# Weepingchestnut/SAVSR

Hardware: AMD Instinct MI355X
Metric: HR Mpixels/sec (Vid4-shape x4, 7-frame window) (higher is better)
Workload: dtype f32 (bf16x3 split products, fp32 accumulate)

## Files before the change

### savsr_amd/csrc/conv_common.hpp

```cpp
#pragma once
#include "common.hpp"

namespace savsr {

struct ConvParams {
    const float* src[SAVSR_MAX_SRC];
    int src_pix[SAVSR_MAX_SRC];
    const unsigned short* wimg;
    const float* bias;
    int act;
    float slope;
    const float* mul_px;
    const float* res1;
    int res1_pix;
    const float* res2;
    int res2_pix;
    float res2_scale;
    float* out;
    int out_pix;
    float* pool;
    int pool_stride;
};

#ifndef SAVSR_CONV_MAX_BATCH
#define SAVSR_CONV_MAX_BATCH 24
#endif
constexpr int CONV_MAX_BATCH = SAVSR_CONV_MAX_BATCH;
constexpr int CONV_WIDE_MIN_TILES = 200;
constexpr int CONV_WIDE_MIN_TILES_TP = 100;
#ifndef SAVSR_CONV_BLOCKS
#define SAVSR_CONV_BLOCKS 256
#endif
constexpr int CONV_PERSISTENT_BLOCKS = SAVSR_CONV_BLOCKS;
#ifndef WY_STRIP
#define WY_STRIP 1
#endif
struct MultiConvParams {
    ConvParams c[CONV_MAX_BATCH];
    int h, w, cout, nchunk, src_ch;
    int nconv, ncob, ntx, nty;
    int wy_tiles, wy_full, wy_strip_l2;
};
static_assert(sizeof(MultiConvParams) <= 4096, "MultiConvParams is passed by value as the conv kernels' argument: at most 4 KB");

int launch_conv_wy(const MultiConvParams& mp, hipStream_t st, bool f16);
int conv_wy_prepare_device();

typedef _Float16 f16x8 __attribute__((ext_vector_type(8)));
typedef _Float16 f16x4 __attribute__((ext_vector_type(4)));

#define SAVSR_GLOBAL __attribute__((address_space(1)))
__device__ __forceinline__ f32x4 ldg4(const float* base, unsigned byte_off) {
    return *(const SAVSR_GLOBAL f32x4*)((const SAVSR_GLOBAL char*)base + byte_off);
}
__device__ __forceinline__ float ldg1(const float* base, unsigned idx) {
    return *((const SAVSR_GLOBAL float*)base + idx);
}
#ifndef CONV_ST
#define CONV_ST 1
#endif
__device__ __forceinline__ void stg4(float* base, unsigned byte_off, const f32x4& v) {
#if CONV_ST == 1
    __builtin_nontemporal_store(v, (SAVSR_GLOBAL f32x4*)((SAVSR_GLOBAL char*)base + byte_off));
#else
    *(SAVSR_GLOBAL f32x4*)((SAVSR_GLOBAL char*)base + byte_off) = v;
#endif
}
__device__ __forceinline__ float vmax_raw(float a, float b) {
    float r;
    asm("v_max_f32 %0, %1, %2" : "=v"(r) : "v"(a), "v"(b));
    return r;
}
__device__ __forceinline__ void stg1(float* base, unsigned idx, float v) {
    *((SAVSR_GLOBAL float*)base + idx) = v;
}

}
```

### savsr_amd/csrc/conv_mfma.hip

```cpp
#include "conv_common.hpp"

#include <type_traits>


#ifndef CONV_BUF
#define CONV_BUF 1
#endif

namespace savsr {

[[maybe_unused]] constexpr int STAMP_BLOCKS = 1024, STAMP_N = 6;
#if defined(SAVSR_DIAG)
#define CONV_HAS_STAMPS 1
__device__ long long g_conv_stamps[STAMP_BLOCKS * STAMP_N];
__device__ int g_conv_stamps_on = 0;
#else
#define CONV_HAS_STAMPS 0
#endif
__device__ __attribute__((aligned(16))) const float g_conv_zero16[4] = {0.f, 0.f, 0.f, 0.f};

__device__ __forceinline__ void stamp(int on, int slot) {
#if CONV_HAS_STAMPS
    if (on == 1 && threadIdx.x == 0 && blockIdx.x < STAMP_BLOCKS)
        g_conv_stamps[blockIdx.x * STAMP_N + slot] = (slot == 5) ? (long long)__builtin_amdgcn_s_memrealtime() : (long long)__builtin_amdgcn_s_memtime();
#endif
}

template <int KS, int NT, int PXT, bool DIAG, bool F16>
__global__ __launch_bounds__(512) void conv_bf16x3_kernel(const MultiConvParams mp) {
    constexpr int TH = CONV_TH * PXT, NTHR = 64 * CONV_TH;
    constexpr int TAPS = KS * KS, HALO = KS / 2;
    constexpr int KC = conv_kc(KS), KSTEPS = KC / 16;
    constexpr int IR = TH + 2 * HALO, IC = CONV_TW + 2 * HALO, NPX = IR * IC;
    constexpr int B_PART = KSTEPS * 2 * NPX;
    constexpr int B_UNITS = 2 * B_PART;
    constexpr int W_UNITS = TAPS * KSTEPS * NT * 2 * 64;
    constexpr int W_IMG = F16 ? W_UNITS / 2 : W_UNITS;
    constexpr int PER = KSTEPS * 4;
    constexpr int B_ITEMS = NPX * PER;
    constexpr int B_IT = (B_ITEMS + NTHR - 1) / NTHR;
    constexpr int W_IT = (W_UNITS + NTHR - 1) / NTHR;
    constexpr int STEPS = TAPS * KSTEPS;
    constexpr int COT = 32 * NT;
    constexpr int EPS = 36;

    extern __shared__ __attribute__((aligned(16))) unsigned char smem_raw[];
    bf16x8* smem = reinterpret_cast<bf16x8*>(smem_raw);
    constexpr bool EP_ALIAS = PXT > 1;
    static_assert(!EP_ALIAS || B_UNITS * 16 >= CONV_TH * 32 * EPS * 4, "aliased epilogue slices must fit one input buffer");

    const int tid = threadIdx.x, lane = tid & 63, wave = tid >> 6, half = lane >> 5, px = lane & 31;
    [[maybe_unused]] const int prio_group = __builtin_amdgcn_readfirstlane(wave >> 2);
    const int tiles_per_cob = mp.ntx * mp.nty;
    const int total = mp.nconv * mp.ncob * tiles_per_cob;
#if CONV_HAS_STAMPS
    const int dbg_all = DIAG ? __builtin_amdgcn_readfirstlane(g_conv_stamps_on) : 0;
#else
    static_assert(!DIAG, "DIAG kernels exist in the instrumented library only");
    const int dbg_all = 0;
#endif
    const int stamps_on = dbg_all & 15;
    const bool dbg_nostage = dbg_all & 16, dbg_nofrag = dbg_all & 32;
    const bool dbg_nost = dbg_all & 64, dbg_nolds = dbg_all & 128;

    f32x4 b_reg[B_IT];
    [[maybe_unused]] const unsigned tid16 = (unsigned)tid * 16u;

    struct TileInfo { int conv, cob, x0, y0, tx, ty; };
    auto decode = [&](int tile) {
        const int cc = tile / tiles_per_cob, rem = tile - cc * tiles_per_cob;
        const int ty = rem / mp.ntx, tx = rem - ty * mp.ntx;
        TileInfo ti;
        ti.conv = cc / mp.ncob;
        ti.cob = cc - ti.conv * mp.ncob;
        ti.x0 = tx * CONV_TW;
        ti.y0 = ty * TH;
        ti.tx = tx;
        ti.ty = ty;
        return ti;
    };
    const int H = mp.h, W = mp.w;
    const float* st_base = nullptr;
    const f32x4* st_w = nullptr;
    int st_pix = 0, st_cb = 0, st_src = 0, st_conv = 0;
#if CONV_BUF
    constexpr unsigned OOB = 0x80000000u;
    unsigned st_voff[B_IT];
    int st_x0 = 0, st_y0 = 0;
    auto stage_offsets = [&]() {
#pragma unroll
        for (int i = 0; i < B_IT; ++i) {
            const int e = tid + i * NTHR;
            const int pl = e / PER, c8 = e - pl * PER;
            const int r = pl / IC, c = pl - r * IC;
            const int gy = st_y0 - HALO + r, gx = st_x0 - HALO + c;
            const bool ok = (e < B_ITEMS) & ((unsigned)gy < (unsigned)H) & ((unsigned)gx < (unsigned)W);
            const unsigned v = (unsigned)((gy * W + gx) * st_pix + c8 * 4) * 4u;
            st_voff[i] = ok ? v : OOB;
        }
    };
    auto uni = [](int v) { return __builtin_amdgcn_readfirstlane(v); };
    auto uni_ptr = [](const float* q) {
        const unsigned long long a = (unsigned long long)(uintptr_t)q;
        const unsigned lo = (unsigned)__builtin_amdgcn_readfirstlane((int)(unsigned)a), hi = (unsigned)__builtin_amdgcn_readfirstlane((int)(unsigned)(a >> 32));
        return (const float*)(uintptr_t)(((unsigned long long)hi << 32) | lo);
    };
#else
    int st_pixoff[B_IT];
    auto uni = [](int v) { return v; };
    auto uni_ptr = [](const float* q) { return q; };
#endif
    auto stage_begin_tile = [&](const TileInfo& ti) {
        st_conv = ti.conv;
        st_src = 0;
        st_cb = 0;
        st_base = uni_ptr(mp.c[ti.conv].src[0]);
        st_pix = uni(mp.c[ti.conv].src_pix[0]);
        st_w = reinterpret_cast<const f32x4*>(mp.c[ti.conv].wimg) + (long long)ti.cob * mp.nchunk * W_IMG;
#if CONV_BUF
        st_x0 = ti.x0;
        st_y0 = ti.y0;
        stage_offsets();
#else
#pragma unroll
        for (int i = 0; i < B_IT; ++i) {
            const int e = tid + i * NTHR;
            int off = -1;
            if (e < B_ITEMS) {
                const int pl = e / PER;
                const int r = pl / IC, c = pl - r * IC;
                const int gy = ti.y0 - HALO + r, gx = ti.x0 - HALO + c;
                if (gy >= 0 && gy < H && gx >= 0 && gx < W) off = gy * W + gx;
            }
            st_pixoff[i] = off;
        }
#endif
    };
    auto stage_advance = [&]() {
        st_cb += KC;
        st_w += W_IMG;
        if (st_cb >= mp.src_ch) {
            st_cb = 0;
            ++st_src;
            st_base = uni_ptr(mp.c[st_conv].src[st_src]);
#if CONV_BUF
            const int pix_new = uni(mp.c[st_conv].src_pix[st_src]);
            if (pix_new != st_pix) { st_pix = pix_new; stage_offsets(); }
#else
            st_pix = mp.c[st_conv].src_pix[st_src];
#endif
        }
    };
    auto issue_w = [&](int g, int wbuf) {
        const int e = tid + g * NTHR;
// ... 513 lines not shown
    asm volatile("s_waitcnt vmcnt(0)" ::: "memory");
    if (stamps_on == 1) {
        __builtin_amdgcn_s_waitcnt(0);
        stamp(stamps_on, 4);
    }
#if CONV_HAS_STAMPS
    if (stamps_on >= 3 && tid == (stamps_on - 3) * 64 && blockIdx.x < STAMP_BLOCKS)
        for (int i = 0; i < 5; ++i) g_conv_stamps[blockIdx.x * STAMP_N + i] = sec[i];
#endif
}

#ifdef SAVSR_DIAG
static int g_conv_diag_host = 0;
#endif

template <int KS, int NT, int PXT>
constexpr size_t conv_lds_bytes() {
    constexpr int TAPS = KS * KS, HALO = KS / 2, KC = conv_kc(KS), KSTEPS = KC / 16;
    constexpr int NPX = (CONV_TH * PXT + 2 * HALO) * (CONV_TW + 2 * HALO);
    return 16ull * 2 * (2 * KSTEPS * 2 * NPX + TAPS * KSTEPS * NT * 2 * 64) + (PXT > 1 ? 0ull : 4ull * CONV_TH * 32 * 36);
}

template <int KS, int NT, int PXT, bool DIAG, bool F16>
static int launch_conv_impl(const MultiConvParams& mp, hipStream_t st) {
    constexpr size_t lds = conv_lds_bytes<KS, NT, PXT>();
    static_assert(lds <= 160 * 1024, "LDS budget");
    if (int rc = ensure_dynamic_lds(reinterpret_cast<const void*>(&conv_bf16x3_kernel<KS, NT, PXT, DIAG, F16>), (int)lds, "conv")) return rc;
    const int total = mp.nconv * mp.ncob * mp.ntx * mp.nty;
    const int grid = total < CONV_PERSISTENT_BLOCKS ? total : CONV_PERSISTENT_BLOCKS;
    hipLaunchKernelGGL((conv_bf16x3_kernel<KS, NT, PXT, DIAG, F16>), dim3(grid), dim3(64 * CONV_TH), lds, st, mp);
    return check_launch("conv_bf16x3_kernel");
}

template <int KS, int NT, int PXT>
static int launch_conv(const MultiConvParams& mp, hipStream_t st, bool f16) {
    if (f16) return launch_conv_impl<KS, NT, PXT, false, true>(mp, st);
#ifdef SAVSR_DIAG
    if (g_conv_diag_host) return launch_conv_impl<KS, NT, PXT, true, false>(mp, st);
#endif
    return launch_conv_impl<KS, NT, PXT, false, false>(mp, st);
}

template <int KS, int NT, int PXT>
static int conv_attr() {
    if (int rc = ensure_dynamic_lds(reinterpret_cast<const void*>(&conv_bf16x3_kernel<KS, NT, PXT, false, false>), (int)conv_lds_bytes<KS, NT, PXT>(), "conv")) return rc;
    return ensure_dynamic_lds(reinterpret_cast<const void*>(&conv_bf16x3_kernel<KS, NT, PXT, false, true>), (int)conv_lds_bytes<KS, NT, PXT>(), "conv");
}
int conv_prepare_device() {
    if (int rc = conv_attr<3, 2, 2>()) return rc;
    if (int rc = conv_attr<3, 2, 1>()) return rc;
    if (int rc = conv_attr<3, 1, 1>()) return rc;
    if (int rc = conv_attr<1, 2, 1>()) return rc;
    if (int rc = conv_attr<1, 2, 2>()) return rc;
    if (int rc = conv_attr<1, 1, 1>()) return rc;
    return conv_wy_prepare_device();
}

}

using namespace savsr;

#if CONV_HAS_STAMPS
extern "C" int savsr_debug_read_conv_stamps(long long* host, int nblocks) {
    if (!host || nblocks < 1 || nblocks > STAMP_BLOCKS) return fail_arg("debug_read_conv_stamps");
    hipError_t e = hipMemcpyFromSymbol(host, HIP_SYMBOL(g_conv_stamps), sizeof(long long) * STAMP_N * nblocks);
    return e == hipSuccess ? 0 : (int)e;
}
#endif
#ifdef SAVSR_DIAG
extern "C" int savsr_debug_conv_stamps(int enable) {
    g_conv_diag_host = enable;
    hipError_t e = hipMemcpyToSymbol(HIP_SYMBOL(g_conv_stamps_on), &enable, sizeof(int));
    return e == hipSuccess ? 0 : (int)e;
}

#endif

extern "C" int savsr_conv_pool_blocks(int h, int w) {
    return ((w + CONV_TW - 1) / CONV_TW) * ((h + CONV_TH - 1) / CONV_TH);
}

extern "C" int64_t savsr_conv_packed_elems(int cout, int cin, int ksize) {
    if (cout <= 0 || cin <= 0 || (ksize != 1 && ksize != 3)) return -1;
    const int kc = conv_kc(ksize), cot = conv_cot(cout);
    if (cin % kc) return -1;
    const int64_t nchunk = cin / kc, ncob = (cout + cot - 1) / cot;
    return ncob * nchunk * ksize * ksize * kc * cot;
}

extern "C" int64_t savsr_conv_pack_index(int cout, int cin, int ksize, int co, int ci, int tap) {
    const int kc = conv_kc(ksize), cot = conv_cot(cout), nt = cot / 32, ksteps = kc / 16;
    const int64_t nchunk = cin / kc;
    const int cob = co / cot, col = co % cot, t = col / 32, row = col % 32;
    const int chunk = ci / kc, cl = ci % kc, ks = cl / 16, kh = (cl % 16) / 8, j = cl % 8;
    const int64_t group = (((int64_t)(cob * nchunk + chunk) * (ksize * ksize) + tap) * ksteps + ks) * nt + t;
    return group * 512 + (kh * 32 + row) * 8 + j;
}

static int fill_params(const savsr_conv_desc* d, ConvParams& p) {
    if (d->ksize != 1 && d->ksize != 3) return fail_arg("conv: ksize must be 1 or 3");
    const int kc = conv_kc(d->ksize);
    if (d->nsrc < 1 || d->nsrc > SAVSR_MAX_SRC || d->src_ch < kc || d->src_ch % kc) return fail_arg("conv: nsrc / src_ch (multiple of 16, or 32 for 1x1)");
    if (d->cin != d->nsrc * d->src_ch) return fail_arg("conv: cin != nsrc*src_ch");
    if (d->h < 1 || d->w < 1 || d->cout < 1) return fail_arg("conv: shape");
    if (!d->wpacked || !d->out) return fail_arg("conv: null weights/out");
    uintptr_t al = reinterpret_cast<uintptr_t>(d->wpacked);
    uintptr_t al_out = reinterpret_cast<uintptr_t>(d->out) | (uintptr_t)(d->out_pix * 4);
    for (int i = 0; i < SAVSR_MAX_SRC; ++i) {
        const bool on = i < d->nsrc;
        if (on && !d->src[i]) return fail_arg("conv: null source");
        p.src[i] = on ? d->src[i] : nullptr;
        p.src_pix[i] = on ? d->src_pix[i] : 0;
        if (on) al |= reinterpret_cast<uintptr_t>(d->src[i]) | (uintptr_t)(d->src_pix[i] * 4);
    }
    if (d->res1) al_out |= reinterpret_cast<uintptr_t>(d->res1) | (uintptr_t)(d->res1_pix * 4);
    if (d->res2) al_out |= reinterpret_cast<uintptr_t>(d->res2) | (uintptr_t)(d->res2_pix * 4);
    if (d->bias) al |= reinterpret_cast<uintptr_t>(d->bias);
    if ((al & 15) || ((al_out & 15) && d->cout >= 4)) {
        set_error("conv: sources / residuals / bias / out / weights must be 16-byte aligned with pixel strides multiple of 4 floats");
        return SAVSR_E_ALIGN;
    }
    p.wimg = reinterpret_cast<const unsigned short*>(d->wpacked);
    p.bias = d->bias; p.act = d->act; p.slope = d->slope;
    p.mul_px = d->mul_px; p.res1 = d->res1; p.res1_pix = d->res1_pix; p.res2 = d->res2; p.res2_pix = d->res2_pix;
    p.res2_scale = d->res2_scale;
    p.out = d->out; p.out_pix = d->out_pix;
    p.pool = d->pool; p.pool_stride = d->pool_stride;
    if (d->pool && (d->cout % 4 || d->pool_stride < d->cout)) return fail_arg("conv: pool needs cout % 4 == 0 and pool_stride >= cout");
    {
        int64_t max_pix = d->out_pix;
        for (int i = 0; i < d->nsrc; ++i) max_pix = d->src_pix[i] > max_pix ? d->src_pix[i] : max_pix;
        if (d->res1 && d->res1_pix > max_pix) max_pix = d->res1_pix;
        if (d->res2 && d->res2_pix > max_pix) max_pix = d->res2_pix;
        if ((int64_t)d->h * d->w * max_pix * 4 >= (int64_t)1 << 31) return fail_arg("conv: tensors of 2 GiB or more are not supported");
    }
    return 0;
}

static void wy_tile_plan(int h, int per, int algo, MultiConvParams& mp) {
    const int left = h % 16, pairs = (left + 1) / 2;
    mp.wy_strip_l2 = pairs <= 1 ? 0 : (pairs <= 2 ? 1 : 2);
    mp.wy_full = mp.wy_tiles = mp.ntx * mp.nty;
    if (WY_STRIP && left > 0 && left <= 8) {
        const int segs = 8 >> mp.wy_strip_l2;
        const int full = mp.ntx * (mp.nty - 1), tiles = full + (mp.ntx + segs - 1) / segs;
        const int wgs = CONV_PERSISTENT_BLOCKS;
        if (WY_STRIP == 2 || (pairs <= 2 && algo == SAVSR_CONV_WINOGRAD_Y_THROUGHPUT) || (per * tiles + wgs - 1) / wgs < (per * mp.wy_tiles + wgs - 1) / wgs) {
            mp.wy_full = full;
            mp.wy_tiles = tiles;
        }
    }
}

extern "C" int64_t savsr_conv_wy_tile_count(int h, int w, int cout, int nconv, int algo) {
    if (h < 1 || w < 1 || cout < 64 || cout % 64 || nconv < 1 || nconv > CONV_MAX_BATCH ||
        (algo != SAVSR_CONV_WINOGRAD_Y && algo != SAVSR_CONV_WINOGRAD_Y_THROUGHPUT)) return -1;
    MultiConvParams mp;
    mp.ncob = cout / 64;
    mp.ntx = (w + CONV_TW - 1) / CONV_TW;
    mp.nty = (h + 15) / 16;
    wy_tile_plan(h, nconv * mp.ncob, algo, mp);
    return (int64_t)nconv * mp.ncob * mp.wy_tiles;
}

extern "C" int savsr_conv2d_max_batch(void) { return CONV_MAX_BATCH; }

static int conv2d_batch(const savsr_conv_desc* descs, int n, void* stream, bool f16) {
    if (!descs) return fail_arg("conv: null descriptor");
    if (n < 1 || n > CONV_MAX_BATCH) return fail_arg("conv: batch size must be 1..24 (savsr_conv2d_max_batch())");
    MultiConvParams mp;
    for (int i = 0; i < n; ++i) {
        const int rc = fill_params(descs + i, mp.c[i]);
        if (rc) return rc;
        const savsr_conv_desc& a = descs[0];
        const savsr_conv_desc& b = descs[i];
        if (b.ksize != a.ksize || b.nsrc != a.nsrc || b.src_ch != a.src_ch || b.h != a.h || b.w != a.w || b.cout != a.cout || b.algo != a.algo)
            return fail_arg("conv: all convs of a batch must share ksize / nsrc / src_ch / h / w / cout / algo");
    }
    for (int i = n; i < CONV_MAX_BATCH; ++i) mp.c[i] = mp.c[0];
    const savsr_conv_desc* d = descs;
    const int cot = conv_cot(d->cout);
    mp.h = d->h; mp.w = d->w; mp.cout = d->cout;
    mp.nchunk = d->cin / conv_kc(d->ksize);
    mp.src_ch = d->src_ch;
    mp.nconv = n;
    mp.ncob = (d->cout + cot - 1) / cot;
    mp.ntx = (d->w + CONV_TW - 1) / CONV_TW;
    mp.nty = (d->h + CONV_TH - 1) / CONV_TH;
    hipStream_t st = static_cast<hipStream_t>(stream);
    if (d->algo == SAVSR_CONV_WINOGRAD_Y || d->algo == SAVSR_CONV_WINOGRAD_Y_THROUGHPUT) {
        if (d->ksize != 3 || d->cout % 64) return fail_arg("conv: algo WINOGRAD_Y needs ksize 3 and cout a multiple of 64");
        mp.nty = (d->h + 15) / 16;
        wy_tile_plan(d->h, n * mp.ncob, d->algo, mp);
        return launch_conv_wy(mp, st, f16);
    }
    if (d->algo != SAVSR_CONV_DIRECT && d->algo != SAVSR_CONV_DIRECT_THROUGHPUT) return fail_arg("conv: unknown algo");
    const bool wide = cot == 64;
    if (d->ksize == 3 && wide) {
        const int nty2 = (d->h + 2 * CONV_TH - 1) / (2 * CONV_TH);
        if (d->cout % 64 == 0 && n * mp.ncob * mp.ntx * nty2 >= (d->algo == SAVSR_CONV_DIRECT_THROUGHPUT ? CONV_WIDE_MIN_TILES_TP : CONV_WIDE_MIN_TILES)) {
            mp.nty = nty2;
            return launch_conv<3, 2, 2>(mp, st, f16);
        }
        return launch_conv<3, 2, 1>(mp, st, f16);
    }
    if (d->ksize == 3) return launch_conv<3, 1, 1>(mp, st, f16);
    if (wide && d->cout % 64 == 0) {
        const int nty2 = (d->h + 2 * CONV_TH - 1) / (2 * CONV_TH);
        if (n * mp.ncob * mp.ntx * nty2 >= (d->algo == SAVSR_CONV_DIRECT_THROUGHPUT ? CONV_WIDE_MIN_TILES_TP : CONV_WIDE_MIN_TILES)) {
            mp.nty = nty2;
            return launch_conv<1, 2, 2>(mp, st, f16);
        }
    }
    return wide ? launch_conv<1, 2, 1>(mp, st, f16) : launch_conv<1, 1, 1>(mp, st, f16);
}

extern "C" int savsr_conv2d_batch(const savsr_conv_desc* descs, int n, void* stream) { return conv2d_batch(descs, n, stream, false); }
extern "C" int savsr_conv2d_batch_f16(const savsr_conv_desc* descs, int n, void* stream) { return conv2d_batch(descs, n, stream, true); }

extern "C" int savsr_conv2d(const savsr_conv_desc* d, void* stream) { return savsr_conv2d_batch(d, 1, stream); }
```

### savsr_amd/csrc/conv_wy.hip

```cpp
#include "conv_common.hpp"

#include <type_traits>

#ifndef WY_STAMPS
#define WY_STAMPS 0
#endif
#ifndef WY_VALU
#define WY_VALU 6
#endif
#ifndef WY_FAST_EPILOGUE
#define WY_FAST_EPILOGUE 1
#endif
#ifndef WY_BUF
#define WY_BUF 1
#endif

namespace savsr {

namespace wy {
constexpr int TH = 16, TW = 32, NTHR = 512, COT = 64;
[[maybe_unused]] constexpr int IC = TW + 2;
#ifndef WY_ICP
#define WY_ICP 36
#endif
constexpr int ICP = WY_ICP;
constexpr int V_PLANE = 2 * ICP;
constexpr int V_WAVE = 2 * 2 * 2 * V_PLANE;
constexpr int W_HALF = 6 * 2 * 2 * 64;
constexpr int W_PHASE = 2 * W_HALF;
constexpr int EPS = 36;
constexpr int LDS_UNITS = 8 * V_WAVE + 2 * W_HALF;
constexpr size_t LDS_BYTES = 16ull * LDS_UNITS + 4ull * 8 * 32 * EPS;
static_assert(LDS_BYTES <= 160 * 1024, "LDS budget");
}

__device__ __attribute__((aligned(16))) const float g_wy_zero16[4] = {0.f, 0.f, 0.f, 0.f};

#if WY_STAMPS
__device__ long long g_wy_stamps[256 * 8 * 8];
#define WY_KSEC(i) (WY_STAMPS == 2 ? 0 : (i))
#define WY_MARK(i) do { const long long t_now = (long long)__builtin_amdgcn_s_memtime(); wy_sec[i] += t_now - wy_prev; wy_prev = t_now; } while (0)
#if WY_STAMPS == 2
#define WY_EMARK(i) WY_MARK(i)
#endif
#else
#define WY_KSEC(i) (i)
#define WY_MARK(i) do { } while (0)
#endif

typedef float f32x2 __attribute__((ext_vector_type(2)));
typedef __bf16 bf16x2 __attribute__((ext_vector_type(2)));
__device__ __forceinline__ void wy_split_store(const f32x4& v, bf16x4* hi_dst, bf16x4* lo_dst) {
    typedef unsigned u32x2 __attribute__((ext_vector_type(2)));
    const f32x2 a[2] = {{v[0], v[1]}, {v[2], v[3]}};
    u32x2 hi, lo;
#pragma unroll
    for (int p = 0; p < 2; ++p) hi[p] = __builtin_bit_cast(unsigned, __builtin_convertvector(a[p], bf16x2));
    asm("" : "+v"(hi[0]), "+v"(hi[1]));
#pragma unroll
    for (int p = 0; p < 2; ++p) {
        const f32x2 back = {__builtin_bit_cast(float, hi[p] << 16), __builtin_bit_cast(float, hi[p] & 0xffff0000u)};
        const f32x2 rest = {a[p][0] - back[0], a[p][1] - back[1]};
        lo[p] = __builtin_bit_cast(unsigned, __builtin_convertvector(rest, bf16x2));
    }
    *hi_dst = __builtin_bit_cast(bf16x4, hi);
    *lo_dst = __builtin_bit_cast(bf16x4, lo);
}
__device__ __forceinline__ void wy_f16_store(const f32x4& v, bf16x4* hi_dst) {
    f16x4 h;
#pragma unroll
    for (int j = 0; j < 4; ++j) h[j] = (_Float16)v[j];
    *hi_dst = __builtin_bit_cast(bf16x4, h);
}

template <bool FAST, bool F16>
__global__ __launch_bounds__(512) void conv_wy_kernel(const MultiConvParams mp) {
    using namespace wy;
    constexpr int WPH = F16 ? W_PHASE / 2 : W_PHASE, WHF = F16 ? W_HALF / 2 : W_HALF;
    extern __shared__ __attribute__((aligned(16))) unsigned char smem_raw[];
    bf16x8* smem = reinterpret_cast<bf16x8*>(smem_raw);
    const int tid = threadIdx.x, lane = tid & 63, wave = tid >> 6, half = lane >> 5, px = lane & 31;
    const int wave_s = __builtin_amdgcn_readfirstlane(wave);
    const int tiles_per_cob = mp.wy_tiles;
    const int total = mp.nconv * mp.ncob * tiles_per_cob;
    const int H = mp.h, W = mp.w;

    struct TileInfo { int conv, cob, x0, y0, tx, ty, strip; };
    auto decode = [&](int tile) {
        const int cc = (int)((unsigned)tile / (unsigned)tiles_per_cob), rem = tile - cc * tiles_per_cob;
        const bool strip = rem >= mp.wy_full;
        const int tyf = (int)((unsigned)rem / (unsigned)mp.ntx);
        const int l2 = strip ? mp.wy_strip_l2 : 3;
        const int ty = strip ? mp.nty - 1 : tyf;
        const int tx = strip ? (rem - mp.wy_full) << (3 - l2) : rem - tyf * mp.ntx;
        const int wx = tx + (wave_s >> l2);
        TileInfo ti;
        ti.conv = (int)((unsigned)cc / (unsigned)mp.ncob);
        ti.cob = cc - ti.conv * mp.ncob;
        ti.x0 = (wx < mp.ntx ? wx : tx) * TW;
        ti.y0 = wx < mp.ntx ? ty * TH - 2 * ((wave_s >> l2) << l2) : mp.nty * TH;
        ti.tx = tx;
        ti.ty = ty;
        ti.strip = strip ? 1 : 0;
        return ti;
    };

    f32x4 d[2][4], dx;
#if !WY_BUF
    int st_pxb[2], st_pxt;
    constexpr int INVALID = -(1 << 30);
#endif
    const float* st_base = nullptr;
    const bf16x8* st_w = nullptr;
    int st_pix = 0, st_cb = 0, st_src = 0, st_conv = 0, st_row0 = 0;
    const int q4 = lane & 3;
#if WY_BUF
    constexpr unsigned OOB = 0x80000000u;
    unsigned st_vcol[2], st_vtail;
    int st_x0 = 0;
    auto stage_cols = [&]() {
#pragma unroll
        for (int r = 0; r < 2; ++r) {
            const int x = st_x0 - 1 + (lane >> 2) + 16 * r;
            const unsigned v = (unsigned)(x * st_pix + 4 * q4) * 4u;
            st_vcol[r] = (unsigned)x < (unsigned)W ? v : OOB;
        }
        const int x = st_x0 - 1 + 32 + ((lane & 7) >> 2), rr = (lane >> 3) & 3, row = st_row0 + rr;
        const unsigned vt = (unsigned)((rr * W + x) * st_pix + 4 * q4) * 4u;
        const bool okt = (lane < 32) & ((unsigned)x < (unsigned)W) & ((unsigned)row < (unsigned)H);
        st_vtail = okt ? vt : OOB;
    };
#endif
#if WY_BUF
    auto uni = [](int v) { return __builtin_amdgcn_readfirstlane(v); };
    auto uni_ptr = [](const float* q) {
        const unsigned long long a = (unsigned long long)(uintptr_t)q;
        const unsigned lo = (unsigned)__builtin_amdgcn_readfirstlane((int)(unsigned)a), hi = (unsigned)__builtin_amdgcn_readfirstlane((int)(unsigned)(a >> 32));
        return (const float*)(uintptr_t)(((unsigned long long)hi << 32) | lo);
    };
#else
    auto uni = [](int v) { return v; };
    auto uni_ptr = [](const float* q) { return q; };
#endif
    auto stage_begin_tile = [&](const TileInfo& ti) {
        st_conv = ti.conv;
        st_src = 0;
        st_cb = 0;
        st_base = uni_ptr(mp.c[ti.conv].src[0]);
        st_pix = uni(mp.c[ti.conv].src_pix[0]);
        st_w = reinterpret_cast<const bf16x8*>(mp.c[ti.conv].wimg) + (long long)ti.cob * mp.nchunk * WPH;
        st_row0 = uni(ti.y0 + 2 * wave_s - 1);
#if WY_BUF
        st_x0 = ti.x0;
        stage_cols();
#else
#pragma unroll
        for (int r = 0; r < 2; ++r) {
            const int x = ti.x0 - 1 + (lane >> 2) + 16 * r;
            st_pxb[r] = (x >= 0 && x < W) ? st_row0 * W + x : INVALID;
        }
        {
            const int x = ti.x0 - 1 + 32 + ((lane & 7) >> 2), row = st_row0 + ((lane >> 3) & 3);
            st_pxt = (lane < 32 && x >= 0 && x < W && row >= 0 && row < H) ? row * W + x : INVALID;
        }
#endif
    };
    auto stage_advance = [&]() {
        st_cb += 16;
        st_w += WPH;
        if (st_cb >= mp.src_ch) {
            st_cb = 0;
            ++st_src;
            st_base = uni_ptr(mp.c[st_conv].src[st_src]);
#if WY_BUF
            const int pix_new = uni(mp.c[st_conv].src_pix[st_src]);
            if (pix_new != st_pix) { st_pix = pix_new; stage_cols(); }
#else
            st_pix = mp.c[st_conv].src_pix[st_src];
#endif
        }
    };
    int st_tile = blockIdx.x, st_chunk = 0;
    auto stage_next = [&]() -> bool {
        if (st_chunk + 1 < mp.nchunk) { ++st_chunk; stage_advance(); return true; }
        if (st_tile + (int)gridDim.x >= total) return false;
        st_tile += gridDim.x;
        st_chunk = 0;
        stage_begin_tile(decode(st_tile));
        return true;
    };
#if WY_BUF
    typedef unsigned u32x4_t __attribute__((ext_vector_type(4)));
    auto row_rsrc = [&](int i, bool whole) {
        const int off = ((st_row0 + i) * W * st_pix + st_cb) * 4;
        const bool row_ok = whole || (st_row0 + i >= 0 && st_row0 + i < H);
        return __builtin_amdgcn_make_buffer_rsrc((void*)((const char*)st_base + off), (short)0, row_ok ? 0x7fffffff : 0, 0x00020000);
    };
    auto issue_row = [&](int r, int i) {
        d[r][i] = __builtin_bit_cast(f32x4, (u32x4_t)__builtin_amdgcn_raw_buffer_load_b128(row_rsrc(i, false), (int)st_vcol[r], 0, 0));
    };
    auto issue_d = [&](int r) {
#pragma unroll
        for (int i = 0; i < 4; ++i) issue_row(r, i);
    };
    auto issue_dx = [&]() { dx = __builtin_bit_cast(f32x4, (u32x4_t)__builtin_amdgcn_raw_buffer_load_b128(row_rsrc(0, true), (int)st_vtail, 0, 0)); };
#else
    auto load_at = [&](int pixel, bool ok) -> f32x4 {
        const SAVSR_GLOBAL float* src = ok ? (const SAVSR_GLOBAL float*)st_base + (pixel * st_pix + st_cb + 4 * q4)
                                           : (const SAVSR_GLOBAL float*)g_wy_zero16;
        return *(const SAVSR_GLOBAL f32x4*)src;
    };
    auto issue_row = [&](int r, int i) {
        const bool row_ok = st_row0 + i >= 0 && st_row0 + i < H;
        d[r][i] = load_at(st_pxb[r] + i * W, row_ok && st_pxb[r] != INVALID);
    };
    auto issue_d = [&](int r) {
#pragma unroll
        for (int i = 0; i < 4; ++i) issue_row(r, i);
    };
    auto issue_dx = [&]() { dx = load_at(st_pxt, st_pxt != INVALID); };
#endif
    bf16x8* vwave = smem + wave * V_WAVE;
    constexpr int PLANE_B = V_PLANE * 16;
    const unsigned vst0 = (unsigned)(wave * V_WAVE + (q4 >> 1) * ICP + (lane >> 2)) * 16u + (unsigned)(q4 & 1) * 8u;
    const unsigned vst_t = (unsigned)(wave * V_WAVE + (q4 >> 1) * ICP + 32 + ((lane & 7) >> 2)) * 16u + (unsigned)(q4 & 1) * 8u;
    auto vptr = [&](unsigned off) { return reinterpret_cast<bf16x4*>(smem_raw + off); };
    auto vstore = [&](const f32x4& v, unsigned off) {
        if constexpr (F16) wy_f16_store(v, vptr(off));
        else wy_split_store(v, vptr(off), vptr(off + PLANE_B));
    };
    auto store_pair = [&](int r, int hf, const f32x4& va, const f32x4& vb) {
        vstore(va, vst0 + (unsigned)(r * 256 + (hf * 2 + 0) * 2 * PLANE_B));
        vstore(vb, vst0 + (unsigned)(r * 256 + (hf * 2 + 1) * 2 * PLANE_B));
    };
    auto store_one = [&](int r, int hf, int vr, const f32x4& v) {
        vstore(v, vst0 + (unsigned)(r * 256 + (hf * 2 + vr) * 2 * PLANE_B));
    };
    auto store_v0 = [&](int r) { store_one(r, 0, 0, d[r][0] - d[r][2]); };
    auto store_v1 = [&](int r) {
        store_one(r, 0, 1, d[r][1] + d[r][2]);
        const f32x4 v2 = d[r][2] - d[r][1], v3 = d[r][1] - d[r][3];
        d[r][0] = v2;
        d[r][1] = v3;
    };
    auto store_v01 = [&](int r) { store_v0(r); store_v1(r); };
    auto store_v23 = [&](int r) { store_pair(r, 1, d[r][0], d[r][1]); };
    const int grp = (lane >> 3) & 3;
    auto tail_value = [&](int hf) -> f32x4 {
        const int partner = hf == 0 ? (grp == 0 ? lane ^ 16 : lane ^ 24) : (grp == 2 ? lane ^ 24 : lane ^ 16);
        f32x4 o;
#pragma unroll
        for (int j = 0; j < 4; ++j) o[j] = __shfl(dx[j], partner, 64);
        return (hf == 0 && grp == 1) ? dx + o : dx - o;
    };
    auto tail_store = [&](int hf, const f32x4& v) {
        const bool mine = lane < 32 && (hf == 0 ? grp < 2 : (grp == 2 || grp == 1));
        const int vr = hf == 0 ? grp : (grp == 2 ? 0 : 1);
        if (mine) {
            vstore(v, vst_t + (unsigned)((hf * 2 + vr) * 2 * PLANE_B));
        }
    };
    auto store_vt01 = [&]() {
        const f32x4 v01 = tail_value(0), v23 = tail_value(1);
        tail_store(0, v01);
        dx = v23;
    };
    auto store_vt23 = [&]() { tail_store(1, dx); };
    bf16x8* wlds = smem + 8 * V_WAVE;
    [[maybe_unused]] const unsigned lane16 = (unsigned)lane * 16u;
    auto issue_w = [&](int j, int hf) {
        const int piece = F16 ? j * 8 + wave_s : wave_s * 3 + j;
        if (F16 && piece >= 12) return;
        const unsigned dst = __builtin_amdgcn_readfirstlane((unsigned)(uintptr_t)(wlds + hf * W_HALF + piece * (F16 ? 128 : 64)));
        unsigned keep;
#if WY_BUF
        asm volatile("s_mov_b32 %0, m0\n\ts_mov_b32 m0, %3\n\ts_nop 0\n\tglobal_load_lds_dwordx4 %1, %2\n\ts_mov_b32 m0, %0"
                     : "=&s"(keep) : "v"(lane16), "s"(st_w + hf * WHF + piece * 64), "s"(dst) : "memory");
#else
        asm volatile("s_mov_b32 %0, m0\n\ts_mov_b32 m0, %2\n\ts_nop 0\n\tglobal_load_lds_dwordx4 %1, off\n\ts_mov_b32 m0, %0"
                     : "=&s"(keep) : "v"(st_w + hf * WHF + piece * 64 + lane), "s"(dst) : "memory");
#endif
    };

    struct FragA { bf16x8 ah, al; };
    struct FragB { bf16x8 bh, bl; };
    const bf16x8* vrd = vwave + half * ICP + px;
    const bf16x8* wrd = wlds + lane;
    auto load_b = [&](int hf, int s, FragB& fr) {
        const int vr = s / 3, kx = s - 3 * vr;
        fr.bh = vrd[((hf * 2 + vr) * 2 + 0) * V_PLANE + kx];
        if (!F16) fr.bl = vrd[((hf * 2 + vr) * 2 + 1) * V_PLANE + kx];
    };
    auto load_a = [&](int hf, int s, int t, FragA& fr) {
        fr.ah = wrd[hf * W_HALF + ((s * 2 + t) * 2 + 0) * 64];
        if (!F16) fr.al = wrd[hf * W_HALF + ((s * 2 + t) * 2 + 1) * 64];
    };

    int tile = blockIdx.x;
#if WY_STAMPS
    long long wy_sec[8] = {0, 0, 0, 0, 0, 0, 0, 0};
    long long wy_prev = (long long)__builtin_amdgcn_s_memtime();
    const long long wy_t0 = wy_prev;
#endif
    FragA fa[2];
    FragB fb[2];
    if (tile < total) {
        stage_begin_tile(decode(tile));
#pragma unroll
        for (int j = 0; j < 3; ++j) issue_w(j, 0);
        issue_d(0);
        issue_d(1);
        issue_dx();
        store_v01(0);
        store_v01(1);
        store_vt01();
    }
    asm volatile("s_waitcnt vmcnt(0)" ::: "memory");
    __syncthreads();
    if (tile < total) { load_b(0, 0, fb[0]); load_a(0, 0, 0, fa[0]); }

    for (; tile < total; tile += gridDim.x) {
        const TileInfo cur = decode(tile);
        const ConvParams& p = mp.c[cur.conv];
        const int cob = cur.cob, x0 = cur.x0, y0 = cur.y0;
        f32x16 acc[4][2];
#pragma unroll
        for (int pz = 0; pz < 4; ++pz)
#pragma unroll
            for (int t = 0; t < 2; ++t)
#pragma unroll
                for (int i = 0; i < 16; ++i) acc[pz][t][i] = 0.f;
        const bool rows_in = y0 + 2 * wave_s < H;
        for (int chunk = 0; chunk < mp.nchunk; ++chunk) {
            auto phase = [&](auto mm) {
                constexpr bool MM = decltype(mm)::value;
                auto pieces = [&](int hf, int s) {
                    if (hf == 0) {
                        if (s == 0) { issue_w(0, 1); issue_w(1, 1); store_v23(0); }
                        if (s == 1) { issue_w(2, 1); stage_next(); issue_row(0, 0); }
                        if (s == 2) { store_v23(1); issue_row(0, 1); issue_row(0, 2); }
                        if (s == 3) { store_vt23(); issue_row(0, 3); issue_row(1, 0); }
                        if (s == 4) { issue_row(1, 1); issue_row(1, 2); }
                        if (s == 5) issue_row(1, 3);
                    } else {
                        if (s < 3) issue_w(s, 0);
                        if (s == 1) store_v0(0);
                        if (s == 2) store_v1(0);
                        if (s == 3) store_v0(1);
                        if (s == 4) store_v1(1);
                        if (s == 5) store_vt01();
                    }
                };
                auto mma3 = [&](int pz, int t, int sb) {
                    const FragA& a = fa[t];
                    const FragB& b = fb[sb];
                    if (MM && F16) {
                        acc[pz][t] = __builtin_amdgcn_mfma_f32_32x32x16_f16(__builtin_bit_cast(f16x8, a.ah), __builtin_bit_cast(f16x8, b.bh), acc[pz][t], 0, 0, 0);
                    } else if (MM) {
                        acc[pz][t] = __builtin_amdgcn_mfma_f32_32x32x16_bf16(a.al, b.bh, acc[pz][t], 0, 0, 0);
                        acc[pz][t] = __builtin_amdgcn_mfma_f32_32x32x16_bf16(a.ah, b.bl, acc[pz][t], 0, 0, 0);
                        acc[pz][t] = __builtin_amdgcn_mfma_f32_32x32x16_bf16(a.ah, b.bh, acc[pz][t], 0, 0, 0);
                    }
                };
#pragma unroll
                for (int hf = 0; hf < 2; ++hf) {
#pragma unroll
                    for (int s = 0; s < 5; ++s) {
                        const int pz = hf * 2 + s / 3;
                        load_a(hf, s, 1, fa[1]);
                        load_b(hf, s + 1, fb[(s + 1) & 1]);
                        __builtin_amdgcn_sched_barrier(0);
                        mma3(pz, 0, s & 1);
                        pieces(hf, s);
                        load_a(hf, s + 1, 0, fa[0]);
                        mma3(pz, 1, s & 1);
                        if (MM && F16) {
#pragma unroll
                            for (int i = 0; i < 2; ++i) {
                                __builtin_amdgcn_sched_group_barrier(0x008, 1, 0);
                                if (i == 1) __builtin_amdgcn_sched_group_barrier(0x100, 1, 0);
                                __builtin_amdgcn_sched_group_barrier(0x002, 3 * WY_VALU, 0);
                                __builtin_amdgcn_sched_group_barrier(0x200, 2, 0);
                                __builtin_amdgcn_sched_group_barrier(0x010, 1, 0);
                            }
                        } else if (MM) {
#pragma unroll
                            for (int i = 0; i < 6; ++i) {
                                __builtin_amdgcn_sched_group_barrier(0x008, 1, 0);
                                if (i == 3) __builtin_amdgcn_sched_group_barrier(0x100, 2, 0);
                                __builtin_amdgcn_sched_group_barrier(0x002, WY_VALU, 0);
                                __builtin_amdgcn_sched_group_barrier(0x200, 1, 0);
                                if (i == 1 || i == 4) __builtin_amdgcn_sched_group_barrier(0x010, 1, 0);
                            }
                        }
                        __builtin_amdgcn_sched_barrier(0);
                    }
                    {
                        const int pz = hf * 2 + 1;
                        load_a(hf, 5, 1, fa[1]);
                        __builtin_amdgcn_sched_barrier(0);
                        mma3(pz, 0, 1);
                        pieces(hf, 5);
                        if (MM) {
#pragma unroll
                            for (int i = 0; i < (F16 ? 1 : 3); ++i) {
                                __builtin_amdgcn_sched_group_barrier(0x008, 1, 0);
                                __builtin_amdgcn_sched_group_barrier(0x002, 10, 0);
                                __builtin_amdgcn_sched_group_barrier(0x200, 1, 0);
                            }
                        }
                        __builtin_amdgcn_sched_barrier(0);
                        WY_MARK(WY_KSEC(hf * 3 + 0));
                        if (hf == 0) asm volatile("s_waitcnt vmcnt(8)" ::: "memory");
                        else asm volatile("s_waitcnt vmcnt(0)" ::: "memory");
                        __syncthreads();
                        WY_MARK(WY_KSEC(hf * 3 + 1));
                        load_b(hf ^ 1, 0, fb[0]);
                        load_a(hf ^ 1, 0, 0, fa[0]);
                        __builtin_amdgcn_sched_barrier(0);
                        mma3(pz, 1, 1);
                        if (hf == 0) issue_dx();
                        __builtin_amdgcn_sched_barrier(0);
                    }
                    WY_MARK(WY_KSEC(hf * 3 + 2));
                }
            };
            auto phase_dead = [&]() {
#pragma unroll
                for (int j = 0; j < 3; ++j) issue_w(j, 1);
                stage_next();
                asm volatile("s_waitcnt vmcnt(0)" ::: "memory");
                __syncthreads();
#pragma unroll
                for (int j = 0; j < 3; ++j) issue_w(j, 0);
                asm volatile("s_waitcnt vmcnt(0)" ::: "memory");
                __syncthreads();
            };
            auto next_tile_rows_in = [&]() {
                if (tile + (int)gridDim.x >= total) return false;
                return decode(tile + (int)gridDim.x).y0 + 2 * wave_s < H;
            };
            if (rows_in) phase(std::true_type{});
            else if (chunk + 1 == mp.nchunk && next_tile_rows_in()) phase(std::false_type{});
            else phase_dead();
        }

        const float* e_bias = p.bias;
        const float* e_mul = p.mul_px;
        const float* e_r1 = p.res1;
        const float* e_r2 = p.res2;
        float* e_out = p.out;
        float* e_pool = p.pool;
        int e_act = p.act, e_opix = p.out_pix, e_r1pix = p.res1_pix, e_r2pix = p.res2_pix;
        float e_slope = p.slope, e_r2s = p.res2_scale;
        asm volatile("" : "+s"(e_bias), "+s"(e_mul), "+s"(e_r1), "+s"(e_r2), "+s"(e_out), "+s"(e_pool));
        asm volatile("" : "+s"(e_act), "+s"(e_opix), "+s"(e_r1pix), "+s"(e_r2pix), "+s"(e_slope), "+s"(e_r2s));
        const bool act_as_max = e_act == SAVSR_ACT_NONE || e_act == SAVSR_ACT_RELU || (e_act == SAVSR_ACT_LRELU && e_slope >= 0.f && e_slope <= 1.f);
        const float slope_eff = e_act == SAVSR_ACT_NONE ? 1.f : (e_act == SAVSR_ACT_RELU ? 0.f : e_slope);
        float* ep_base = reinterpret_cast<float*>(smem + LDS_UNITS);
        float* ep = ep_base + wave * (32 * EPS);
        const int c4 = lane & 7;
        const bool x_inside = x0 + TW <= W;
        const float* zero16 = (const float*)g_wy_zero16;
        const float* b_base = e_bias ? e_bias : zero16;
        const unsigned b_off = e_bias ? 4u * (unsigned)(cob * COT + 4 * c4) : 0u, b_step = e_bias ? 128u : 0u;
        f32x4 bias4[2];
#pragma unroll
        for (int t = 0; t < 2; ++t) bias4[t] = ldg4(b_base, b_off + (unsigned)t * b_step);
        const float* r1_base = e_r1 ? e_r1 : zero16;
        constexpr int RR = 2;
        f32x4 rr[RR][4];
        auto load_r1 = [&](int r, int t, f32x4 (&dst)[4]) {
            const int y = y0 + 2 * wave_s + r;
            const int co = cob * COT + 32 * t + 4 * c4;
            const unsigned off0 = 4u * (unsigned)((y * W + x0 + (lane >> 3)) * e_r1pix + co), ustride = 32u * (unsigned)e_r1pix;
            const bool row_ok = e_r1 && y < H;
#pragma unroll
            for (int i = 0; i < 4; ++i) {
                const bool ok = row_ok && (x_inside || x0 + (lane >> 3) + 8 * i < W);
                dst[i] = ldg4(r1_base, ok ? off0 + (unsigned)i * ustride : 0u);
            }
        };
#pragma unroll
        for (int gi = 0; gi < RR; ++gi) load_r1(gi / 2, gi % 2, rr[gi]);
        __builtin_amdgcn_sched_barrier(0);
#pragma unroll
        for (int t = 0; t < 2; ++t)
#pragma unroll
            for (int i = 0; i < 16; ++i) {
                const float m1 = acc[1][t][i], m2 = acc[2][t][i];
                acc[0][t][i] = (acc[0][t][i] + m1) + m2;
                acc[3][t][i] = (m1 - m2) - acc[3][t][i];
            }
        f32x4 psum[2][2];
#ifdef WY_EMARK
        asm volatile("" :: "v"(acc[0][0][0]), "v"(acc[3][1][15]));
        WY_EMARK(1);
#endif
#pragma unroll
        for (int r = 0; r < 2; ++r) {
            const int y = y0 + 2 * wave_s + r;
            const int pbase = y * W + x0 + (lane >> 3);
#pragma unroll
            for (int t = 0; t < 2; ++t) {
                psum[r][t] = f32x4{0.f, 0.f, 0.f, 0.f};
                const int gi = r * 2 + t;
                if (y >= H) {
                    asm volatile("" :: "v"(bias4[t]), "v"(rr[gi % RR][0]), "v"(rr[gi % RR][1]), "v"(rr[gi % RR][2]), "v"(rr[gi % RR][3]));
                    if (gi + RR < 4) load_r1((gi + RR) / 2, (gi + RR) % 2, rr[gi % RR]);
                    continue;
                }
                const f32x16& a = r == 0 ? acc[0][t] : acc[3][t];
#pragma unroll
                for (int g = 0; g < 4; ++g) {
                    const f32x4 v = {a[4 * g], a[4 * g + 1], a[4 * g + 2], a[4 * g + 3]};
                    *reinterpret_cast<f32x4*>(ep + px * EPS + 8 * g + 4 * half) = v;
                }
                const int co = cob * COT + 32 * t + 4 * c4;
                const f32x4 b4 = bias4[t];
                const unsigned ooff0 = 4u * (unsigned)(pbase * e_opix + co), ostride = 32u * (unsigned)e_opix;
                f32x4 ps = {0.f, 0.f, 0.f, 0.f};
#pragma unroll
                for (int ih = 0; ih < 2; ++ih) {
                    const int p0 = pbase + 16 * ih;
                    const bool ok0 = x_inside || x0 + (lane >> 3) + 16 * ih < W, ok1 = x_inside || x0 + (lane >> 3) + 16 * ih + 8 < W;
                    f32x4 v[2];
#pragma unroll
                    for (int i = 0; i < 2; ++i) {
                        const f32x4 a4 = *reinterpret_cast<const f32x4*>(ep + ((lane >> 3) + 16 * ih + 8 * i) * EPS + 4 * c4);
                        v[i] = a4 + b4;
                    }
                    if constexpr (FAST) {
#pragma unroll
                        for (int i = 0; i < 2; ++i) {
                            const f32x4 sv = v[i] * slope_eff;
#pragma unroll
                            for (int q = 0; q < 4; ++q) v[i][q] = vmax_raw(v[i][q], sv[q]);
                        }
                    } else if (e_act == SAVSR_ACT_NONE) {
                    } else if (act_as_max) {
#pragma unroll
                        for (int i = 0; i < 2; ++i) {
                            const f32x4 sv = v[i] * slope_eff;
#pragma unroll
                            for (int q = 0; q < 4; ++q) v[i][q] = vmax_raw(v[i][q], sv[q]);
                        }
                    } else if (e_act == SAVSR_ACT_LRELU) {
#pragma unroll
                        for (int i = 0; i < 2; ++i)
#pragma unroll
                            for (int q = 0; q < 4; ++q) v[i][q] = v[i][q] > 0.f ? v[i][q] : v[i][q] * e_slope;
                    } else if (e_act == SAVSR_ACT_SIGMOID) {
#pragma unroll
                        for (int i = 0; i < 2; ++i)
#pragma unroll
                            for (int q = 0; q < 4; ++q) v[i][q] = sigmoidf_(v[i][q]);
                    }
                    if (!FAST && e_mul) {
                        const float m0 = ok0 ? ldg1(e_mul, (unsigned)p0) : 0.f, m1 = ok1 ? ldg1(e_mul, (unsigned)(p0 + 8)) : 0.f;
#pragma unroll
                        for (int q = 0; q < 4; ++q) { v[0][q] *= m0; v[1][q] *= m1; }
                    }
                    v[0] += rr[gi % RR][2 * ih];
                    v[1] += rr[gi % RR][2 * ih + 1];
                    if (!FAST && e_r2) {
                        f32x4 ra = {0.f, 0.f, 0.f, 0.f}, rb = {0.f, 0.f, 0.f, 0.f};
                        if (ok0) ra = ldg4(e_r2, 4u * (unsigned)(p0 * e_r2pix + co));
                        if (ok1) rb = ldg4(e_r2, 4u * (unsigned)((p0 + 8) * e_r2pix + co));
#pragma unroll
                        for (int q = 0; q < 4; ++q) { v[0][q] += e_r2s * ra[q]; v[1][q] += e_r2s * rb[q]; }
                    }
#pragma unroll
                    for (int i = 0; i < 2; ++i) {
                        if (i == 0 ? ok0 : ok1) {
                            stg4(e_out, ooff0 + (unsigned)(2 * ih + i) * ostride, v[i]);
                            if (e_pool) ps += v[i];
                        }
                    }
                }
                psum[r][t] = ps;
#ifdef WY_EMARK
                WY_EMARK(2 + gi);
#endif
                if (gi + RR < 4) load_r1((gi + RR) / 2, (gi + RR) % 2, rr[gi % RR]);
            }
        }
        if (e_pool) {
#pragma unroll
            for (int r = 0; r < 2; ++r)
#pragma unroll
                for (int t = 0; t < 2; ++t)
#pragma unroll
                    for (int o = 8; o < 64; o <<= 1) {
// ... 81 lines not shown
```

Baseline: 144.5.

## Partition Winograd-Y tiles per XCD with source-grouped walk order

```diff
diff --git a/savsr_amd/csrc/conv_common.hpp b/savsr_amd/csrc/conv_common.hpp
--- a/savsr_amd/csrc/conv_common.hpp
+++ b/savsr_amd/csrc/conv_common.hpp
@@ -35,11 +35,17 @@
 #ifndef WY_STRIP
 #define WY_STRIP 1
 #endif
+#ifndef WY_ORDER
+#define WY_ORDER 1
+#endif
 struct MultiConvParams {
     ConvParams c[CONV_MAX_BATCH];
     int h, w, cout, nchunk, src_ch;
     int nconv, ncob, ntx, nty;
     int wy_tiles, wy_full, wy_strip_l2;
+    int wy_run;
+    unsigned wy_div[8];
+    int wy_lo[9];
 };
 static_assert(sizeof(MultiConvParams) <= 4096, "MultiConvParams is passed by value as the conv kernels' argument: at most 4 KB");
 
diff --git a/savsr_amd/csrc/conv_mfma.hip b/savsr_amd/csrc/conv_mfma.hip
--- a/savsr_amd/csrc/conv_mfma.hip
+++ b/savsr_amd/csrc/conv_mfma.hip
@@ -1,5 +1,6 @@
 #include "conv_common.hpp"
 
+#include <algorithm>
 #include <type_traits>
 
 
@@ -819,6 +820,37 @@
     }
 }
 
+static int wy_shares(int units, int unit, int grid, int (&lo)[9]) {
+    int worst = 0, cum = 0;
+    lo[0] = 0;
+    for (int x = 0; x < 8; ++x) {
+        const int n = (grid >> 3) + (x < (grid & 7) ? 1 : 0);
+        cum += n;
+        lo[x + 1] = (int)((int64_t)units * cum / grid) * unit;
+        if (n) worst = std::max(worst, (lo[x + 1] - lo[x] + n - 1) / n);
+    }
+    return worst;
+}
+static void wy_walk_plan(MultiConvParams& mp) {
+    int g = 1;
+    for (int c = mp.nconv; c > 1 && g == 1; --c) {
+        if (mp.nconv % c) continue;
+        bool same = true;
+        for (int i = 0; i < mp.nconv && same; ++i) same = mp.c[i].src[0] == mp.c[i - i % c].src[0] && mp.c[i].src_pix[0] == mp.c[i - i % c].src_pix[0];
+        if (same) g = c;
+    }
+    const int total = mp.nconv * mp.ncob * mp.wy_tiles;
+    const int grid = total < CONV_PERSISTENT_BLOCKS ? total : CONV_PERSISTENT_BLOCKS;
+    mp.wy_run = g;
+    const int members = g * mp.ncob;
+    const int divisors[4] = {members, mp.wy_tiles, std::max(1, mp.wy_full / mp.ntx), mp.ncob};
+    for (int i = 0; i < 4; ++i) {
+        mp.wy_div[2 * i] = (unsigned)divisors[i];
+        mp.wy_div[2 * i + 1] = divisors[i] == 1 ? 0xffffffffu : (unsigned)(((uint64_t)1 << 32) / (unsigned)divisors[i]);
+    }
+    if (wy_shares(total / members, members, grid, mp.wy_lo) > (total + grid - 1) / grid) wy_shares(total, 1, grid, mp.wy_lo);
+}
+
 extern "C" int64_t savsr_conv_wy_tile_count(int h, int w, int cout, int nconv, int algo) {
     if (h < 1 || w < 1 || cout < 64 || cout % 64 || nconv < 1 || nconv > CONV_MAX_BATCH ||
         (algo != SAVSR_CONV_WINOGRAD_Y && algo != SAVSR_CONV_WINOGRAD_Y_THROUGHPUT)) return -1;
@@ -859,6 +891,7 @@
         if (d->ksize != 3 || d->cout % 64) return fail_arg("conv: algo WINOGRAD_Y needs ksize 3 and cout a multiple of 64");
         mp.nty = (d->h + 15) / 16;
         wy_tile_plan(d->h, n * mp.ncob, d->algo, mp);
+        wy_walk_plan(mp);
         return launch_conv_wy(mp, st, f16);
     }
     if (d->algo != SAVSR_CONV_DIRECT && d->algo != SAVSR_CONV_DIRECT_THROUGHPUT) return fail_arg("conv: unknown algo");
diff --git a/savsr_amd/csrc/conv_wy.hip b/savsr_amd/csrc/conv_wy.hip
--- a/savsr_amd/csrc/conv_wy.hip
+++ b/savsr_amd/csrc/conv_wy.hip
@@ -1,5 +1,6 @@
 #include "conv_common.hpp"
 
+#include <cstddef>
 #include <type_traits>
 
 #ifndef WY_STAMPS
@@ -81,22 +82,56 @@
     bf16x8* smem = reinterpret_cast<bf16x8*>(smem_raw);
     const int tid = threadIdx.x, lane = tid & 63, wave = tid >> 6, half = lane >> 5, px = lane & 31;
     const int wave_s = __builtin_amdgcn_readfirstlane(wave);
-    const int tiles_per_cob = mp.wy_tiles;
+    [[maybe_unused]] const int tiles_per_cob = mp.wy_tiles;
+    const int H = mp.h, W = mp.w;
+#if WY_ORDER
+    const int wy_x = (int)blockIdx.x & 7;
+    const int wy_step = ((int)gridDim.x >> 3) + (wy_x < ((int)gridDim.x & 7) ? 1 : 0);
+    const int wy_first = mp.wy_lo[wy_x] + ((int)blockIdx.x >> 3);
+#define WY_T_FIRST wy_first
+#define WY_T_STEP wy_step
+    const int total = mp.wy_lo[wy_x + 1];
+    auto divmod = [](int n, int dv, unsigned rcp, int& rem) {
+        int q = (int)__umulhi((unsigned)n, rcp);
+        rem = n - q * dv;
+        const bool up = rem >= dv;
+        rem = up ? rem - dv : rem;
+        return up ? q + 1 : q;
+    };
+#else
     const int total = mp.nconv * mp.ncob * tiles_per_cob;
-    const int H = mp.h, W = mp.w;
+#define WY_T_FIRST ((int)blockIdx.x)
+#define WY_T_STEP ((int)gridDim.x)
+#endif
 
     struct TileInfo { int conv, cob, x0, y0, tx, ty, strip; };
     auto decode = [&](int tile) {
+        TileInfo ti;
+#if WY_ORDER
+        typedef unsigned u32x8_t __attribute__((ext_vector_type(8)));
+        u32x8_t dv;
+        asm volatile("s_load_dwordx8 %0, %1, %2\n\ts_waitcnt lgkmcnt(0)" : "=s"(dv) : "s"(__builtin_amdgcn_kernarg_segment_ptr()), "i"(offsetof(MultiConvParams, wy_div)) : "memory");
+        int mem, rem, tyf;
+        const int site = divmod(tile, (int)dv[0], dv[1], mem);
+        const int run = divmod(site, (int)dv[2], dv[3], rem);
+        const bool strip = rem >= mp.wy_full;
+        const int txf = divmod(rem, (int)dv[4], dv[5], tyf);
+        const int l2 = strip ? mp.wy_strip_l2 : 3;
+        const int ty = strip ? mp.nty - 1 : tyf;
+        const int tx = strip ? (rem - mp.wy_full) << (3 - l2) : txf;
+        const int cr = divmod(mem, (int)dv[6], dv[7], ti.cob);
+        ti.conv = run * mp.wy_run + cr;
+#else
         const int cc = (int)((unsigned)tile / (unsigned)tiles_per_cob), rem = tile - cc * tiles_per_cob;
         const bool strip = rem >= mp.wy_full;
         const int tyf = (int)((unsigned)rem / (unsigned)mp.ntx);
         const int l2 = strip ? mp.wy_strip_l2 : 3;
         const int ty = strip ? mp.nty - 1 : tyf;
         const int tx = strip ? (rem - mp.wy_full) << (3 - l2) : rem - tyf * mp.ntx;
-        const int wx = tx + (wave_s >> l2);
-        TileInfo ti;
         ti.conv = (int)((unsigned)cc / (unsigned)mp.ncob);
         ti.cob = cc - ti.conv * mp.ncob;
+#endif
+        const int wx = tx + (wave_s >> l2);
         ti.x0 = (wx < mp.ntx ? wx : tx) * TW;
         ti.y0 = wx < mp.ntx ? ty * TH - 2 * ((wave_s >> l2) << l2) : mp.nty * TH;
         ti.tx = tx;
@@ -180,11 +215,11 @@
 #endif
         }
     };
-    int st_tile = blockIdx.x, st_chunk = 0;
+    int st_tile = WY_T_FIRST, st_chunk = 0;
     auto stage_next = [&]() -> bool {
         if (st_chunk + 1 < mp.nchunk) { ++st_chunk; stage_advance(); return true; }
-        if (st_tile + (int)gridDim.x >= total) return false;
-        st_tile += gridDim.x;
+        if (st_tile + WY_T_STEP >= total) return false;
+        st_tile += WY_T_STEP;
         st_chunk = 0;
         stage_begin_tile(decode(st_tile));
         return true;
@@ -296,7 +331,7 @@
         if (!F16) fr.al = wrd[hf * W_HALF + ((s * 2 + t) * 2 + 1) * 64];
     };
 
-    int tile = blockIdx.x;
+    int tile = WY_T_FIRST;
 #if WY_STAMPS
     long long wy_sec[8] = {0, 0, 0, 0, 0, 0, 0, 0};
     long long wy_prev = (long long)__builtin_amdgcn_s_memtime();
@@ -319,7 +354,7 @@
     __syncthreads();
     if (tile < total) { load_b(0, 0, fb[0]); load_a(0, 0, 0, fa[0]); }
 
-    for (; tile < total; tile += gridDim.x) {
+    for (; tile < total; tile += WY_T_STEP) {
         const TileInfo cur = decode(tile);
         const ConvParams& p = mp.c[cur.conv];
         const int cob = cur.cob, x0 = cur.x0, y0 = cur.y0;
@@ -437,8 +472,8 @@
                 __syncthreads();
             };
             auto next_tile_rows_in = [&]() {
-                if (tile + (int)gridDim.x >= total) return false;
-                return decode(tile + (int)gridDim.x).y0 + 2 * wave_s < H;
+                if (tile + WY_T_STEP >= total) return false;
+                return decode(tile + WY_T_STEP).y0 + 2 * wave_s < H;
             };
             if (rows_in) phase(std::true_type{});
             else if (chunk + 1 == mp.nchunk && next_tile_rows_in()) phase(std::false_type{});
```

After: 145.8, median of 6. No clear change (+0.9%).
